# JARVIS-MoCap/JARVIS-HybridNet

Hardware: AMD Instinct MI355X
Metric: multi-view frames/s (12cam 1280x1024, 23kpt, 64^3 grid) (higher is better)
Workload: dtype f32; 1 GPU; BASELINE configs[2]: HybridNet 12-camera 1280x1024, 23 kpts, 64^3 grid, small/small; cameras=12, joints=23, grid=64, streams=3, parallelism=single GPU, 3 time batches in flight on 3 HIP streams, hipgraph=False

## Files before the change

### include/jarvis_hip.h

```cpp
#ifndef JARVIS_HIP_H
#define JARVIS_HIP_H
#include <stdint.h>

#ifdef __cplusplus
extern "C" {
#endif

#define JH_ABI_VERSION 4

const char* jh_last_error(void);
int jh_abi_version(void);

#define JH_PRECISION_DEFAULT (-1)
#define JH_PRECISION_F32 0
#define JH_PRECISION_BF16X3 1
#define JH_PRECISION_BF16X3_WIDE 2
int jh_set_precision(int mode);
int jh_get_precision(void);

typedef struct jh_params jh_params;
int jh_params_create(jh_params** out);
int jh_params_set(jh_params* p, const char* key, const float* host, int64_t numel);
void jh_params_destroy(jh_params* p);

typedef struct jh_efftrack jh_efftrack;
int jh_efftrack_create(const jh_params* p, const char* prefix, int model_size, int joints, int n,
                       int h, int w, int want_res1, jh_efftrack** out);
int jh_efftrack_forward(jh_efftrack* net, const float* x_dev, float* res1_dev, float* res2_dev,
                        void* stream);
int64_t jh_efftrack_launches(const jh_efftrack* net);
void jh_efftrack_destroy(jh_efftrack* net);

typedef struct jh_v2v jh_v2v;
int jh_v2v_create(const jh_params* p, const char* prefix, int joints, int t, int g, jh_v2v** out);
int jh_v2v_forward(jh_v2v* net, const float* x_dev, float* y_dev, void* stream);
void jh_v2v_destroy(jh_v2v* net);

int64_t jh_reproject_workspace_bytes(int cams, int joints, int hs, int grid_size);
int jh_reproject_forward(const float* heatmaps_padded_dev, int cams, int joints, int hs,
                         const int32_t* center3d_dev, const int32_t* center_hm_dev,
                         const float* cam_dev, const float* intr_dev, const float* dist_dev,
                         int grid_size, float grid_spacing, float* vol_dev, int32_t* idx_dev,
                         void* workspace_dev, int64_t workspace_bytes, void* stream);

int64_t jh_softargmax_workspace_bytes(int t, int joints, int gh);
int jh_softargmax(const float* v2v_out_dev, int t, int joints, int gh, float grid_spacing,
                  float roi_cube_size, const int32_t* center3d_dev, float* heatmap_final_dev,
                  float* points_dev, float* conf_dev, void* workspace_dev, int64_t workspace_bytes,
                  void* stream);

int jh_reproject_point(const float* points_dev, int npoints, int cams, const float* cam_dev,
                       const float* intr_dev, const float* dist_dev, float* uv_dev, void* stream);
int64_t jh_reconstruct_workspace_bytes(int cams);
int jh_reconstruct_point(const float* points2d_dev, const float* maxvals_dev, int cams,
                         const float* cam_dev, const float* intr_dev, const float* dist_dev,
                         float* point3d_dev, void* workspace_dev, int64_t workspace_bytes,
                         void* stream);

typedef struct jh_predictor jh_predictor;
typedef struct {
  int32_t num_cameras, num_joints;
  int32_t center_size;
  int32_t bbox;
  float roi_cube_size;
  float grid_spacing;
  int32_t center_model, kp_model;
  int32_t img_h, img_w;
  int32_t time_batch;
  int32_t time_batch_3d;
  int32_t cam_lo, cam_n;
  float mean[3], std[3];
  int32_t precision;
} jh_predictor_config;

int jh_predictor_create(const jh_params* center_params, const jh_params* hybrid_params,
                        const jh_predictor_config* cfg, jh_predictor** out);
void jh_predictor_destroy(jh_predictor* pr);
int64_t jh_predictor_launches(const jh_predictor* pr);
int64_t jh_predictor_device_bytes(const jh_predictor* pr);
int jh_predictor_precision(const jh_predictor* pr);

int jh_predictor_set_calibration(jh_predictor* pr, const float* cam_dev, const float* intr_dev,
                                 const float* dist_dev, void* stream);
int jh_predictor_set_calibration_frames(jh_predictor* pr, const float* cam_dev ,
                                        const float* intr_dev , const float* dist_dev ,
                                        void* stream);

int jh_predictor_set_centers(jh_predictor* pr, const float* centers_dev , void* stream);

int jh_predictor_stage_center(jh_predictor* pr, const float* frames_dev, float* det_dev,
                              void* stream);
int jh_predictor_stage_keypoints(jh_predictor* pr, const float* frames_dev,
                                 const float* det_all_dev, float* heat_dev, void* stream);
int jh_predictor_stage_3d(jh_predictor* pr, const float* heat_all_dev, int t0, float* points_dev,
                          float* conf_dev, int32_t* valid_dev, void* stream);
int jh_predictor_stage_keypoints_gathered(jh_predictor* pr, const void* frames_dev, int frames_u8,
                                          const float* det_gathered_dev, int n_blocks,
                                          float* heat_dev, void* stream);
int jh_predictor_stage_3d_blocks(jh_predictor* pr, const float* heat_blocks_dev, int n_blocks,
                                 int frames_per_block, int t_off, int t0, float* points_dev,
                                 float* conf_dev, int32_t* valid_dev, void* stream);
int jh_predictor_forward(jh_predictor* pr, const float* frames_dev, float* points_dev,
                         float* conf_dev, int32_t* valid_dev, void* stream);
int jh_predictor_set_graph_replay(jh_predictor* pr, int on);
int jh_predictor_graph_replay(const jh_predictor* pr);
int jh_predictor_stage_center_u8(jh_predictor* pr, const uint8_t* frames_dev, float* det_dev,
                                 void* stream);
int jh_predictor_stage_keypoints_u8(jh_predictor* pr, const uint8_t* frames_dev,
                                    const float* det_all_dev, float* heat_dev, void* stream);
int jh_predictor_forward_u8(jh_predictor* pr, const uint8_t* frames_dev, float* points_dev,
                            float* conf_dev, int32_t* valid_dev, void* stream);

#define JH_FRAME_RGB_F32 0
#define JH_FRAME_BGR_U8 1
#define JH_FRAME_I420 2
#define JH_FRAME_NV12 3
int jh_predictor_forward_yuv(jh_predictor* pr, const uint8_t* frames_dev, int format, float* points_dev,
                             float* conf_dev, int32_t* valid_dev, void* stream);

// ... 163 lines not shown
```

### jarvis-hybridnet_amd/_native.py

```python
import ctypes
import math
import os
from typing import NamedTuple

import torch

_HERE = os.path.dirname(os.path.abspath(__file__))
LIB_PATH = os.environ.get("JH_LIBRARY_PATH") or os.path.join(_HERE, "libjarvis_hip.so")
_lib = None

c_void_p, c_int, c_float, c_int64 = ctypes.c_void_p, ctypes.c_int, ctypes.c_float, ctypes.c_int64
c_char_p = ctypes.c_char_p


class PredictorConfig(ctypes.Structure):
    _fields_ = [("num_cameras", ctypes.c_int32), ("num_joints", ctypes.c_int32),
                ("center_size", ctypes.c_int32), ("bbox", ctypes.c_int32),
                ("roi_cube_size", c_float), ("grid_spacing", c_float),
                ("center_model", ctypes.c_int32), ("kp_model", ctypes.c_int32),
                ("img_h", ctypes.c_int32), ("img_w", ctypes.c_int32),
                ("time_batch", ctypes.c_int32), ("time_batch_3d", ctypes.c_int32),
                ("cam_lo", ctypes.c_int32),
                ("cam_n", ctypes.c_int32), ("mean", c_float * 3), ("std", c_float * 3),
                ("precision", ctypes.c_int32)]


class YuvSurfaceStruct(ctypes.Structure):
    _fields_ = [("image_stride", ctypes.c_int64), ("y_offset", ctypes.c_int64), ("y_pitch", ctypes.c_int64),
                ("u_offset", ctypes.c_int64), ("v_offset", ctypes.c_int64), ("c_pitch", ctypes.c_int64),
                ("c_step", ctypes.c_int32), ("matrix", ctypes.c_int32), ("range", ctypes.c_int32),
                ("reserved", ctypes.c_int32)]


assert ctypes.sizeof(YuvSurfaceStruct) == 64


class SensorSurfaceStruct(ctypes.Structure):
    _fields_ = [("image_stride", ctypes.c_int64), ("offset", ctypes.c_int64), ("pitch", ctypes.c_int64),
                ("pattern", ctypes.c_int32), ("reserved", ctypes.c_int32)]


assert ctypes.sizeof(SensorSurfaceStruct) == 32

class OpOperand(ctypes.Structure):
    _fields_ = [("in_sums_host", c_void_p), ("in_act", ctypes.c_int32), ("latency_class", ctypes.c_int32),
                ("want_stats", ctypes.c_int32), ("se_c", ctypes.c_int32), ("se_s", ctypes.c_int32),
                ("se_inv_hw", c_float), ("se_wr_host", c_void_p), ("se_br_host", c_void_p),
                ("se_we_host", c_void_p), ("se_be_host", c_void_p), ("se_pool_host", c_void_p)]


assert ctypes.sizeof(OpOperand) == 72

class SubjectsParamsStruct(ctypes.Structure):
    _fields_ = [("max_subjects", ctypes.c_int32), ("max_peaks", ctypes.c_int32), ("nms_radius", ctypes.c_int32),
                ("min_views", ctypes.c_int32), ("min_peak", c_float), ("max_error_px", c_float)]


assert ctypes.sizeof(SubjectsParamsStruct) == 24

ABI_VERSION = 4
assert ctypes.sizeof(PredictorConfig) == 84

_WORKSPACES = {}


def workspace(nbytes, device):
    key = (str(device), torch.cuda.current_stream(device).cuda_stream)
    bufs = _WORKSPACES.setdefault(key, [])
    if not bufs or bufs[-1].numel() < nbytes:
        bufs.append(torch.empty((max(int(nbytes), 256),), dtype=torch.uint8, device=device))
    return bufs[-1]


_SIGS = {
    "jh_last_error": (c_char_p, []),
    "jh_abi_version": (c_int, []),
    "jh_set_precision": (c_int, [c_int]),
    "jh_get_precision": (c_int, []),
    "jh_params_create": (c_int, [ctypes.POINTER(c_void_p)]),
    "jh_params_set": (c_int, [c_void_p, c_char_p, c_void_p, c_int64]),
    "jh_params_destroy": (None, [c_void_p]),
    "jh_efftrack_create": (c_int, [c_void_p, c_char_p, c_int, c_int, c_int, c_int, c_int, c_int,
                                   ctypes.POINTER(c_void_p)]),
    "jh_efftrack_forward": (c_int, [c_void_p, c_void_p, c_void_p, c_void_p, c_void_p]),
    "jh_efftrack_launches": (c_int64, [c_void_p]),
    "jh_efftrack_destroy": (None, [c_void_p]),
    "jh_v2v_create": (c_int, [c_void_p, c_char_p, c_int, c_int, c_int, ctypes.POINTER(c_void_p)]),
    "jh_v2v_forward": (c_int, [c_void_p, c_void_p, c_void_p, c_void_p]),
    "jh_v2v_destroy": (None, [c_void_p]),
    "jh_reproject_workspace_bytes": (c_int64, [c_int, c_int, c_int, c_int]),
    "jh_reproject_forward": (c_int, [c_void_p, c_int, c_int, c_int, c_void_p, c_void_p, c_void_p,
                                     c_void_p, c_void_p, c_int, c_float, c_void_p, c_void_p,
                                     c_void_p, c_int64, c_void_p]),
    "jh_softargmax_workspace_bytes": (c_int64, [c_int, c_int, c_int]),
    "jh_softargmax": (c_int, [c_void_p, c_int, c_int, c_int, c_float, c_float, c_void_p, c_void_p,
                              c_void_p, c_void_p, c_void_p, c_int64, c_void_p]),
    "jh_softargmax_spread_workspace_bytes": (c_int64, [c_int, c_int, c_int]),
    "jh_softargmax_spread": (c_int, [c_void_p, c_int, c_int, c_int, c_float, c_float, c_void_p, c_void_p,
                                     c_void_p, c_void_p, c_void_p, c_void_p, c_void_p, c_void_p, c_int64, c_void_p]),
    "jh_predictor_set_spread": (c_int, [c_void_p, c_int]),
    "jh_predictor_get_spread": (c_int, [c_void_p, c_void_p, c_void_p, c_void_p, c_void_p]),
    "jh_predictor_debug_v2v": (c_int, [c_void_p, c_void_p, c_void_p]),
    "jh_reproject_point": (c_int, [c_void_p, c_int, c_int, c_void_p, c_void_p, c_void_p, c_void_p,
                                   c_void_p]),
    "jh_reconstruct_workspace_bytes": (c_int64, [c_int]),
    "jh_reconstruct_point": (c_int, [c_void_p, c_void_p, c_int, c_void_p, c_void_p, c_void_p,
                                     c_void_p, c_void_p, c_int64, c_void_p]),
    "jh_predictor_create": (c_int, [c_void_p, c_void_p, ctypes.POINTER(PredictorConfig),
                                    ctypes.POINTER(c_void_p)]),
    "jh_predictor_destroy": (None, [c_void_p]),
    "jh_predictor_set_graph_replay": (c_int, [c_void_p, c_int]),
    "jh_predictor_graph_replay": (c_int, [c_void_p]),
    "jh_predictor_launches": (c_int64, [c_void_p]),
    "jh_predictor_device_bytes": (c_int64, [c_void_p]),
    "jh_predictor_precision": (c_int, [c_void_p]),
    "jh_predictor_set_calibration": (c_int, [c_void_p, c_void_p, c_void_p, c_void_p, c_void_p]),
    "jh_predictor_set_calibration_frames": (c_int, [c_void_p, c_void_p, c_void_p, c_void_p, c_void_p]),
    "jh_predictor_set_centers": (c_int, [c_void_p, c_void_p, c_void_p]),
    "jh_predictor_stage_center": (c_int, [c_void_p, c_void_p, c_void_p, c_void_p]),
    "jh_predictor_stage_keypoints": (c_int, [c_void_p, c_void_p, c_void_p, c_void_p, c_void_p]),
    "jh_predictor_stage_3d": (c_int, [c_void_p, c_void_p, c_int, c_void_p, c_void_p, c_void_p,
                                      c_void_p]),
    "jh_predictor_stage_keypoints_gathered": (c_int, [c_void_p, c_void_p, c_int, c_void_p, c_int, c_void_p,
                                                      c_void_p]),
    "jh_predictor_stage_3d_blocks": (c_int, [c_void_p, c_void_p, c_int, c_int, c_int, c_int, c_void_p,
                                             c_void_p, c_void_p, c_void_p]),
    "jh_profile_begin": (c_int, []),
    "jh_profile_end": (c_int, [ctypes.POINTER(c_int)]),
    "jh_profile_get": (c_int, [c_int, c_char_p, c_int, ctypes.POINTER(ctypes.c_double),
                               ctypes.POINTER(ctypes.c_double), ctypes.POINTER(ctypes.c_double)]),
    "jh_predictor_forward": (c_int, [c_void_p, c_void_p, c_void_p, c_void_p, c_void_p, c_void_p]),
    "jh_predictor_stage_center_u8": (c_int, [c_void_p, c_void_p, c_void_p, c_void_p]),
    "jh_predictor_stage_keypoints_u8": (c_int, [c_void_p, c_void_p, c_void_p, c_void_p, c_void_p]),
    "jh_predictor_forward_u8": (c_int, [c_void_p, c_void_p, c_void_p, c_void_p, c_void_p, c_void_p]),
    "jh_predictor_forward_yuv": (c_int, [c_void_p, c_void_p, c_int, c_void_p, c_void_p, c_void_p, c_void_p]),
    "jh_yuv_surface_check": (c_int, [ctypes.POINTER(YuvSurfaceStruct), c_int, c_int]),
    "jh_predictor_forward_surface": (c_int, [c_void_p, c_void_p, ctypes.POINTER(YuvSurfaceStruct), c_void_p, c_void_p,
                                             c_void_p, c_void_p, c_void_p]),
    "jh_predictor2d_forward_surface": (c_int, [c_void_p, c_void_p, ctypes.POINTER(YuvSurfaceStruct), c_void_p,
                                               c_void_p, c_void_p, c_void_p]),
    "jh_op_yuv_surface_to_bgr": (c_int, [c_void_p, ctypes.POINTER(YuvSurfaceStruct), c_int, c_int, c_int, c_void_p,
                                         c_void_p]),
    "jh_sensor_surface_check": (c_int, [ctypes.POINTER(SensorSurfaceStruct), c_int, c_int]),
    "jh_predictor_forward_sensor": (c_int, [c_void_p, c_void_p, ctypes.POINTER(SensorSurfaceStruct), c_void_p, c_void_p,
                                            c_void_p, c_void_p, c_void_p]),
    "jh_predictor2d_forward_sensor": (c_int, [c_void_p, c_void_p, ctypes.POINTER(SensorSurfaceStruct), c_void_p,
                                              c_void_p, c_void_p, c_void_p]),
    "jh_op_sensor_to_bgr": (c_int, [c_void_p, ctypes.POINTER(SensorSurfaceStruct), c_int, c_int, c_int, c_void_p,
                                    c_void_p]),
    "jh_predictor_forward_masked": (c_int, [c_void_p, c_void_p, c_int, c_void_p, c_void_p, c_void_p, c_void_p,
                                            c_void_p]),
    "jh_predictor_forward_images": (c_int, [c_void_p, ctypes.POINTER(c_void_p), c_int, c_int,
                                            ctypes.POINTER(YuvSurfaceStruct), ctypes.POINTER(SensorSurfaceStruct),
                                            c_void_p, c_void_p, c_void_p, c_void_p, c_void_p]),
    "jh_predictor2d_forward_images": (c_int, [c_void_p, ctypes.POINTER(c_void_p), c_int, c_int,
                                              ctypes.POINTER(YuvSurfaceStruct), ctypes.POINTER(SensorSurfaceStruct),
                                              c_void_p, c_void_p, c_void_p, c_void_p]),
    "jh_predictor_stage_keypoints_masked": (c_int, [c_void_p, c_void_p, c_int, c_void_p, c_void_p, c_void_p,
                                                    c_void_p]),
    "jh_predictor_stage_3d_masked": (c_int, [c_void_p, c_void_p, c_int, c_void_p, c_void_p, c_void_p, c_void_p,
                                             c_void_p]),
    "jh_predictor_debug_mask": (c_int, [c_void_p, c_void_p, c_void_p, c_void_p]),
    "jh_predictor_views2d": (c_int, [c_void_p, c_void_p, c_int] + [c_void_p] * 8),
    "jh_subjects_params_check": (c_int, [ctypes.POINTER(SubjectsParamsStruct)]),
    "jh_op_center_peaks": (c_int, [c_void_p, c_int, c_int, c_int, c_int, ctypes.POINTER(SubjectsParamsStruct), c_void_p,
                                   c_void_p, c_void_p]),
    "jh_op_associate_subjects": (c_int, [c_void_p, c_int, c_int, c_void_p, c_void_p, c_void_p, c_int, c_void_p,
                                         c_float, c_float, ctypes.POINTER(SubjectsParamsStruct), c_void_p, c_void_p,
                                         c_void_p, c_void_p, c_void_p]),
    "jh_predictor_detect_subjects": (c_int, [c_void_p, c_void_p, ctypes.POINTER(c_void_p), c_int, c_int,
                                             ctypes.POINTER(YuvSurfaceStruct), ctypes.POINTER(SensorSurfaceStruct),
                                             c_void_p, ctypes.POINTER(SubjectsParamsStruct), c_void_p, c_void_p,
# ... 372 lines not shown
```

### jarvis-hybridnet_amd/csrc/api.hip

```cpp
#include <cstring>
#include <memory>
#include "../../include/jarvis_hip.h"
#include <cstdlib>
#include "nets.h"
#include "bifpn_node.h"
#include "views2d.h"
#include "subjects.h"

namespace jh {
static thread_local std::string g_err;
void set_error(const std::string& msg) { g_err = msg; }
}

using namespace jh;

struct jh_params { ParamMap map; };
struct jh_efftrack { EffTrackPlan plan; };
struct jh_v2v { V2VPlan plan; };

namespace {

struct Scratch {
  std::vector<void*> ptrs;
  ~Scratch() { for (void* p : ptrs) (void)hipFree(p); }
// ... 93 lines not shown
  if (i < count) table[i] = c.p[i];
}
__global__ void copy_out_kernel(const float* __restrict__ gp, const float* __restrict__ gc,
                                const int* __restrict__ gv, float* __restrict__ points,
                                float* __restrict__ conf, int* __restrict__ valid, int n_pts, int n_conf,
                                int n_valid) {
  const int i = blockIdx.x * blockDim.x + threadIdx.x;
  if (i < n_pts) points[i] = gp[i];
  if (i < n_conf) conf[i] = gc[i];
  if (valid && i < n_valid) valid[i] = gv[i];
}

__global__ void pack_det_kernel(const float* __restrict__ pts2d, const float* __restrict__ maxvals,
                                float* __restrict__ det, int C) {
  const int c = threadIdx.x;
  if (c < C) {
    det[c * 3 + 0] = pts2d[c];
    det[c * 3 + 1] = pts2d[C + c];
    det[c * 3 + 2] = maxvals[c];
  }
}

}

extern "C" {

const char* jh_last_error(void) { return g_err.c_str(); }
int jh_abi_version(void) { return JH_ABI_VERSION; }

int jh_set_precision(int mode) {
  JH_REQUIRE(mode == JH_PRECISION_F32 || mode == JH_PRECISION_BF16X3 || mode == JH_PRECISION_BF16X3_WIDE,
             "unknown precision mode");
  set_precision_mode(mode);
  return 0;
}
int jh_get_precision(void) { return precision_mode(); }

int jh_params_create(jh_params** out) {
  *out = new jh_params();
  return 0;
}
int jh_params_set(jh_params* p, const char* key, const float* host, int64_t numel) {
  JH_REQUIRE(p && key && host && numel >= 0, "bad argument");
  p->map[key] = std::vector<float>(host, host + numel);
  return 0;
}
void jh_params_destroy(jh_params* p) { delete p; }

int jh_efftrack_create(const jh_params* p, const char* prefix, int model_size, int joints, int n,
                       int h, int w, int want_res1, jh_efftrack** out) {
  JH_REQUIRE(p && out, "bad argument");
  std::unique_ptr<jh_efftrack> net(new jh_efftrack());
  if (net->plan.build(p->map, prefix ? prefix : "", model_size, joints, n, h, w, want_res1 != 0)) return 1;
  *out = net.release();
  return 0;
}
int jh_efftrack_forward(jh_efftrack* net, const float* x_dev, float* res1_dev, float* res2_dev,
                        void* stream) {
  hipStream_t s = static_cast<hipStream_t>(stream);
  JH_REQUIRE(net && x_dev && res2_dev, "bad argument");
  JH_REQUIRE(!res1_dev || net->plan.res1.p, "res1 requested from a network created with want_res1 = 0");
  if (launch_to_channel_last(x_dev, net->plan.input, s)) return 1;
  if (net->plan.run(s)) return 1;
  if (res1_dev && launch_from_channel_last(net->plan.res1, res1_dev, s)) return 1;
  return launch_from_channel_last(net->plan.heat, res2_dev, s);
}
int64_t jh_efftrack_launches(const jh_efftrack* net) { return (int64_t)net->plan.launches(); }
void jh_efftrack_destroy(jh_efftrack* net) { delete net; }

int jh_v2v_create(const jh_params* p, const char* prefix, int joints, int t, int g, jh_v2v** out) {
  JH_REQUIRE(p && out, "bad argument");
  std::unique_ptr<jh_v2v> net(new jh_v2v());
  if (net->plan.build(p->map, prefix ? prefix : "", joints, t, g)) return 1;
  *out = net.release();
  return 0;
}
int jh_v2v_forward(jh_v2v* net, const float* x_dev, float* y_dev, void* stream) {
  hipStream_t s = static_cast<hipStream_t>(stream);
  if (launch_to_channel_last(x_dev, net->plan.input, s)) return 1;
  if (net->plan.run(s)) return 1;
  return launch_from_channel_last(net->plan.output, y_dev, s);
}
void jh_v2v_destroy(jh_v2v* net) { delete net; }

int64_t jh_reproject_workspace_bytes(int cams, int joints, int hs, int grid_size) {
  Carver c(nullptr, 0);
  ReproWs w;
  return (int64_t)carve_reproject(c, cams, joints, hs, grid_size, &w);
}

int jh_reproject_forward(const float* heatmaps_padded_dev, int cams, int joints, int hs,
                         const int32_t* center3d_dev, const int32_t* center_hm_dev,
                         const float* cam_dev, const float* intr_dev, const float* dist_dev,
                         int grid_size, float grid_spacing, float* vol_dev, int32_t* idx_dev,
                         void* workspace_dev, int64_t workspace_bytes, void* stream) {
  hipStream_t s = static_cast<hipStream_t>(stream);
  JH_REQUIRE(workspace_dev && workspace_bytes >= 0, "workspace (see jh_reproject_workspace_bytes)");
  JH_REQUIRE(grid_size > 0 && grid_size % 2 == 0, "grid size must be even");
  Carver c(workspace_dev, (size_t)workspace_bytes);
  ReproWs w;
  carve_reproject(c, cams, joints, hs, grid_size, &w);
  JH_REQUIRE(c.fits(), "workspace smaller than jh_reproject_workspace_bytes()");
  if (launch_to_channel_last(heatmaps_padded_dev, w.heat, s)) return 1;
  if (launch_reproject(Calib{cam_dev, intr_dev, dist_dev, 0}, center3d_dev, center_hm_dev, w.heat.p, w.coarse,
                       w.vol.p, idx_dev, 1, cams, grid_size, grid_spacing, hs, w.heat.Cp,
                       1, 0, nullptr, s)) return 1;
  return launch_from_channel_last(w.vol, vol_dev, s);
}

int64_t jh_softargmax_workspace_bytes(int t, int joints, int gh) {
  Carver c(nullptr, 0);
  SoftWs w;
  return (int64_t)carve_softargmax(c, t, joints, gh, &w);
}

int jh_softargmax(const float* v2v_out_dev, int t, int joints, int gh, float grid_spacing,
                  float roi_cube_size, const int32_t* center3d_dev, float* heatmap_final_dev,
                  float* points_dev, float* conf_dev, void* workspace_dev, int64_t workspace_bytes,
                  void* stream) {
  hipStream_t s = static_cast<hipStream_t>(stream);
  JH_REQUIRE(workspace_dev && workspace_bytes >= 0, "workspace (see jh_softargmax_workspace_bytes)");
  Carver c(workspace_dev, (size_t)workspace_bytes);
  SoftWs w;
  carve_softargmax(c, t, joints, gh, &w);
  JH_REQUIRE(c.fits(), "workspace smaller than jh_softargmax_workspace_bytes()");
  if (launch_to_channel_last(v2v_out_dev, w.x, s)) return 1;
  return launch_softargmax(w.x.p, center3d_dev, w.partial, w.pmax, points_dev, conf_dev,
                           heatmap_final_dev, t, joints, w.x.Cp, gh, grid_spacing, roi_cube_size, s);
}

int64_t jh_softargmax_spread_workspace_bytes(int t, int joints, int gh) {
  Carver c(nullptr, 0);
  SoftWs w;
  SoftargmaxSpread sp;
  carve_softargmax(c, t, joints, gh, &w);
  return (int64_t)carve_spread(c, t, w.x.Cp, &sp);
}

int jh_softargmax_spread(const float* v2v_out_dev, int t, int joints, int gh, float grid_spacing,
                         float roi_cube_size, const int32_t* center3d_dev, float* heatmap_final_dev,
                         float* points_dev, float* conf_dev, float* cov_dev, float* peak_dev, float* mass_dev,
                         void* workspace_dev, int64_t workspace_bytes, void* stream) {
  hipStream_t s = static_cast<hipStream_t>(stream);
  JH_REQUIRE(workspace_dev && workspace_bytes >= 0, "workspace (see jh_softargmax_spread_workspace_bytes)");
  JH_REQUIRE(cov_dev && peak_dev && mass_dev, "jh_softargmax_spread: null output pointer");
  Carver c(workspace_dev, (size_t)workspace_bytes);
  SoftWs w;
  SoftargmaxSpread sp;
  carve_softargmax(c, t, joints, gh, &w);
  carve_spread(c, t, w.x.Cp, &sp);
  JH_REQUIRE(c.fits(), "workspace smaller than jh_softargmax_spread_workspace_bytes()");
  sp.cov = cov_dev; sp.peak = peak_dev; sp.mass = mass_dev;
  if (launch_to_channel_last(v2v_out_dev, w.x, s)) return 1;
  return launch_softargmax(w.x.p, center3d_dev, w.partial, w.pmax, points_dev, conf_dev,
                           heatmap_final_dev, t, joints, w.x.Cp, gh, grid_spacing, roi_cube_size, s, &sp);
}

int jh_reproject_point(const float* points_dev, int npoints, int cams, const float* cam_dev,
                       const float* intr_dev, const float* dist_dev, float* uv_dev, void* stream) {
  return launch_project_points(points_dev, cam_dev, intr_dev, dist_dev, uv_dev, npoints, cams,
                               static_cast<hipStream_t>(stream));
}

int64_t jh_reconstruct_workspace_bytes(int cams) {
  Carver c(nullptr, 0);
  ReconWs w;
// ... 1408 lines not shown
```

### jarvis-hybridnet_amd/csrc/jh_common.h

```cpp
#pragma once
#include <hip/hip_runtime.h>
#include <cstdlib>
#include <cstdint>
#include <cstdio>
#include <cstring>
#include <string>
#include <vector>

namespace jh {

constexpr int kWave = 64;

#define JH_ENV_KNOB(name) ([]() -> int { static const int v = [] { const char* e = getenv(name); return e ? atoi(e) : -1; }(); return v; }())

inline int round_up(int v, int m) { return (v + m - 1) / m * m; }
inline int cpad(int c) { return round_up(c, 8); }

void set_error(const std::string& msg);
#define JH_CHECK_HIP(expr)                                                     \
  do {                                                                         \
    hipError_t _e = (expr);                                                    \
    if (_e != hipSuccess) {                                                    \
      jh::set_error(std::string(#expr) + ": " + hipGetErrorString(_e));        \
      return 1;                                                                \
// ... 181 lines not shown
__device__ __forceinline__ double exact_read(const double* src) { return (src[0] + src[1]) + src[2]; }
__device__ __forceinline__ void stat_add(double* st, float s1, float s2) {
  exact_add(st, (double)s1);
  exact_add(st + kLimbs, (double)s2);
}
__device__ __forceinline__ void exact_add_rounded(double* dst, double p) {
  const double a = fabs(p);
  double q;
  int slot;
  if (a < 0x1p5) { q = rint(p * 0x1p35) * 0x1p-35; slot = 2; }
  else if (a < 0x1p15) { q = rint(p * 0x1p25) * 0x1p-25; slot = 1; }
  else { q = rint(p * 0x1p15) * 0x1p-15; slot = 0; }
  if (q != 0.0) unsafeAtomicAdd(dst + slot, q);
}
__device__ __forceinline__ void stat_add(double* st, double s1, double s2) {
  exact_add_rounded(st, s1);
  exact_add_rounded(st + kLimbs, s2);
}
__device__ __forceinline__ void stat_acc(double& s1, double& s2, float v) {
  const double d = (double)v;
  s1 += d;
  s2 = fma(d, d, s2);
}
#endif

#if defined(__HIPCC__)
__device__ __forceinline__ unsigned xcd_linear(unsigned L, unsigned total) {
  const unsigned q = total >> 3, r = total & 7u, x = L & 7u, s = L >> 3;
  return x < r ? x * (q + 1) + s : r * (q + 1) + (x - r) * q + s;
}
__device__ __forceinline__ unsigned fd_div(unsigned x, const FastDiv& f) { return (__umulhi(x, f.mul) + x) >> f.shift; }
__device__ __forceinline__ BlockId xcd_block(const FastDiv& fgx, const FastDiv& fgy) {
  const unsigned gx = gridDim.x, gy = gridDim.y, gz = gridDim.z;
  const unsigned L = blockIdx.x + gx * (blockIdx.y + gy * blockIdx.z);
  const unsigned l = xcd_linear(L, gx * gy * gz);
  BlockId b;
  const unsigned l1 = fd_div(l, fgx);
  b.x = l - l1 * gx;
  b.z = fd_div(l1, fgy);
  b.y = l1 - b.z * gy;
  return b;
}
__device__ __forceinline__ BlockId xcd_block() {
  const unsigned gx = gridDim.x, gy = gridDim.y, gz = gridDim.z;
  const unsigned L = blockIdx.x + gx * (blockIdx.y + gy * blockIdx.z);
  unsigned l = xcd_linear(L, gx * gy * gz);
  BlockId b;
  b.x = l % gx; l /= gx;
  b.y = l % gy;
  b.z = l / gy;
  return b;
}
#endif

#if defined(__HIPCC__)
__device__ __forceinline__ float sum_xor16(float s) {
  const auto r = __builtin_amdgcn_permlane16_swap(__float_as_uint(s), __float_as_uint(s), false, false);
  return __uint_as_float(r[0]) + __uint_as_float(r[1]);
}
__device__ __forceinline__ float sum_xor32(float s) {
  const auto r = __builtin_amdgcn_permlane32_swap(__float_as_uint(s), __float_as_uint(s), false, false);
  return __uint_as_float(r[0]) + __uint_as_float(r[1]);
}
__device__ __forceinline__ double sum_xor16(double s) {
  const unsigned lo = (unsigned)__double2loint(s), hi = (unsigned)__double2hiint(s);
  const auto a = __builtin_amdgcn_permlane16_swap(lo, lo, false, false);
  const auto b = __builtin_amdgcn_permlane16_swap(hi, hi, false, false);
  return __hiloint2double((int)b[0], (int)a[0]) + __hiloint2double((int)b[1], (int)a[1]);
}
__device__ __forceinline__ double sum_xor32(double s) {
  const unsigned lo = (unsigned)__double2loint(s), hi = (unsigned)__double2hiint(s);
  const auto a = __builtin_amdgcn_permlane32_swap(lo, lo, false, false);
  const auto b = __builtin_amdgcn_permlane32_swap(hi, hi, false, false);
  return __hiloint2double((int)b[0], (int)a[0]) + __hiloint2double((int)b[1], (int)a[1]);
}
__device__ __forceinline__ float silu_fast(float v) { return v * __builtin_amdgcn_rcpf(1.f + __expf(-v)); }
#endif

struct NodeArgs;
int launch_bifpn_node(const NodeArgs& a, hipStream_t s);
int pack_wino_weights(int cin, int cout, const float* w, const float* b, ConvWeights* out);
int launch_conv3d_wino(const ConvWeights& w, const Act& x, const Act& y, double* stats, hipStream_t s,
                       const InNorm* in, int variant, const int* tables);
inline unsigned short bf16_rne(float f) {
  unsigned u;
  std::memcpy(&u, &f, 4);
  u += 0x7fffu + ((u >> 16) & 1u);
  return (unsigned short)(u >> 16);
}
inline float bf16_to_f32(unsigned short h) {
  const unsigned u = (unsigned)h << 16;
  float f;
  std::memcpy(&f, &u, 4);
  return f;
}
int pack_bf16x3_weights(int cin, int cout, const float* w, const float* b, ConvWeights* out);
int launch_conv3d_bf16x3(const ConvWeights& w, const Act& x, const Act& y, double* stats, hipStream_t s,
                         const InNorm* in);
int pack_deconv4_bf16x3_weights(int cin, int cout, const float* w, ConvWeights* out);
bool deconv4_bf16x3_eligible(int cout);
int launch_deconv4_bf16x3(const ConvWeights& w, const Act& x, const Act& y, hipStream_t s, const InNorm* in);
bool conv_bf16x3_eligible(const ConvDesc& d);
int pack_conv_bf16x3_weights(const ConvDesc& d, const float* w, const float* b, ConvWeights* out);
int launch_conv_bf16x3(const ConvDesc& d, const ConvWeights& w, const Act& x, const Act& y, double* stats,
                       hipStream_t s, const InNorm* in);
int precision_mode();
void set_precision_mode(int m);
void pack_stem_weights(const float* w_host, float* packed, int cout);
int launch_stem_conv(const Act& x, const float* w_dev, const Act& y, double* stats, hipStream_t s);
struct StemSource;
int launch_stem_conv_src(const StemSource& src, const Act& x, const float* w_dev, const Act& y, double* stats,
                         hipStream_t s);
int launch_deconv_c1(const Act& x, const double* stats, float inv_cnt, int in_act, const float* w,
                     const Act& y, hipStream_t s);

int launch_zero(void* p, size_t bytes, hipStream_t s);

int launch_to_channel_last(const float* src, const Act& dst, hipStream_t s);
int launch_from_channel_last(const Act& src, float* dst, hipStream_t s);

}
```

### jarvis-hybridnet_amd/csrc/nets.h

```cpp
#pragma once
#include <deque>
#include <functional>
#include <map>
#include <string>
#include <vector>
#include "jh_common.h"
#include "conv_layer.h"
#include "preprocess.h"

namespace jh {

int launch_reproject(const Calib& cal, const int* center3d, const int* center_hm, const float* heat, float2* coarse,
                     float* vol, int* idx_out, int T, int C, int G, float spacing, int hs, int Jp, int heat_pad,
                     int div255, const unsigned char* mask, hipStream_t s, const HeatLayout* layout = nullptr);
int launch_preprocess_resize(const void* frames, const FrameSource& src, float* out, int N, int H, int W, int S,
                             const float* mean, const float* stdv, hipStream_t s,
                             const void* const* frames_cell = nullptr);
int launch_preprocess_crop(const void* frames, const FrameSource& src, const int* center_hm, float* out, int T,
                           int Cloc, int C, int cam0, int H, int W, int B, const float* mean,
                           const float* stdv, hipStream_t s, const void* const* frames_cell = nullptr);
int launch_frames_to_bgr(const void* frames, const FrameSource& src, unsigned char* out, int N, int H, int W,
                         hipStream_t s);
int launch_center_argmax(const float* heat, float* det, int N, int Hh, int Wh, int Cp,
                         hipStream_t s);
// ... 21 lines not shown
                      int Gh, float spacing, float roi, hipStream_t s, const SoftargmaxSpread* spread = nullptr);

typedef std::map<std::string, std::vector<float>> ParamMap;

class Plan {
 public:
  ~Plan();
  int run(hipStream_t s);
  size_t launches() const { return ops_.size(); }
  size_t device_bytes() const { return bytes_; }
  int precision = precision_mode();
  int norm_block_kb = 0;

 protected:
  int alloc(void** p, size_t bytes);
  int new_act(int N, int D, int H, int W, int C, Act* out);
  size_t scratch(size_t doubles);
  int finish();
  double* sc(size_t off) const { return arena_ + off; }
  int upload(const std::vector<float>& host, float** dev);
  int get(const ParamMap& pm, const std::string& key, size_t numel, const float** out);

  struct Op { std::function<int(hipStream_t)> fn; std::string name; double flops, bytes; };
  std::vector<Op> ops_;
  void push(const std::string& name, double flops, double bytes, std::function<int(hipStream_t)> fn) {
    ops_.push_back(Op{std::move(fn), name, flops, bytes});
  }
  std::vector<void*> owned_;
  std::deque<ConvLayer> layers_;
  std::vector<ConvWeights> convs_;
  double* arena_ = nullptr;
  size_t arena_doubles_ = 0;
  size_t bytes_ = 0;

  int add_conv(const ParamMap& pm, const ConvDesc& d, const std::string& wkey,
               const std::string& bkey, bool transposed, const Act& x, const Act& y,
               const float* gate, bool want_stats, size_t* stats_off, long in_stats_off = -1,
               float in_inv = 0.f, int in_act = 0, const SeGate* se = nullptr, long se_pool_off = -1);
  void add_norm(const Act& x, size_t stats_off, int act, const float* r1, const float* r2,
                float* y, long pool_off, long r1_stats_off = -1);
};

struct Ref {
  Act a;
  long st = -1;
  float inv = 0.f;
  int act = 0;
};

class EffTrackPlan : public Plan {
 public:
  int build(const ParamMap& pm, const std::string& prefix, int size, int J, int N, int H, int W,
            bool want_res1 = false);
  bool stem_fusable = false;
  StemSource stem_src;
  void set_stem_traffic(double bytes);
  int stem_channels() const { return stem_ch_; }
  int node_rows = -1;
  Act input;
  Act heat;
  Act res1;
  int J = 0;
  int stem_op_ = -1, stem_ch_ = 16;

 private:
  int mbconv(const ParamMap& pm, const std::string& p, int stage, int k, int stride, int cin,
             int cout, int expand, Ref* x, Ref* out);
  void materialise(Ref* x);
  int lateral(const ParamMap& pm, const std::string& p, int cout, const Ref& x, Ref* out);
  int pool(const Ref& x, Ref* out);
  int node(const ParamMap& pm, const std::string& conv_prefix, int n_in, const Ref* ins,
           const int* modes, const float* w, int act, const Act& like, int cout, Ref* out,
           Ref* pooled = nullptr);
};

class V2VPlan : public Plan {
 public:
  int build(const ParamMap& pm, const std::string& prefix, int J, int T, int G);
  Act input;
  Act output;

 private:
  int res_block(const ParamMap& pm, const std::string& p, int c, const Act& x, const float* extra,
                Act* out, long x_stats = -1);
};

}
```

### jarvis-hybridnet_amd/csrc/nets.hip

```cpp
#include <cmath>
#include <cstring>
#include <cstdlib>
#include "nets.h"
#include "bifpn_node.h"

namespace jh {

Profiler& profiler() {
  static Profiler p;
  return p;
}
void Profiler::begin(const std::string& name, double flops, double bytes, hipStream_t s) {
  ProfRec r{name, flops, bytes, nullptr, nullptr, 0.f};
  (void)hipEventCreate(&r.e0);
  (void)hipEventCreate(&r.e1);
  (void)hipEventRecord(r.e0, s);
  recs.push_back(r);
}
void Profiler::end(hipStream_t s) { (void)hipEventRecord(recs.back().e1, s); }
int Profiler::finish() {
  JH_CHECK_HIP(hipDeviceSynchronize());
  for (auto& r : recs) {
    if (!r.e0) continue;
    JH_CHECK_HIP(hipEventElapsedTime(&r.ms, r.e0, r.e1));
// ... 390 lines not shown
      if (lateral(pm, p + "p5_down_channel", Wf, feats[2], &p5_in)) return 1;
      if (lateral(pm, p + "p4_down_channel_2", Wf, feats[1], &p4_in2)) return 1;
      if (lateral(pm, p + "p5_down_channel_2", Wf, feats[2], &p5_in2)) return 1;
    } else {
      p3_in = p3; p4_in = p4; p5_in = p5; p6_in = p6; p7_in = p7;
      p4_in2 = p4; p5_in2 = p5;
    }
    auto fnode = [&](const char* wname, int n_in, const Ref* ins, const int* modes, const Ref& like,
                     const char* conv, Ref* out, Ref* pooled = nullptr) -> int {
      const float* wp = nullptr;
      if (get(pm, p + wname, n_in, &wp)) return 1;
      float w[3];
      fuse_weights(wp, n_in, w);
      return node(pm, p + conv + ".", n_in, ins, modes, w, ACT_SILU, like.a, Wf, out, pooled);
    };
    const int m_up[2] = {FUSE_SAME, FUSE_UP2};
    const int m_dn3[3] = {FUSE_SAME, FUSE_SAME, FUSE_POOL2};
    const int m_dn2[2] = {FUSE_SAME, FUSE_POOL2};
    Ref p6_up, p5_up, p4_up, p3_out, p4_out, p5_out, p6_out, p7_out;
    { const Ref in[2] = {p6_in, p7_in}; if (fnode("p6_w1", 2, in, m_up, p6_in, "conv6_up", &p6_up)) return 1; }
    { const Ref in[2] = {p5_in, p6_up}; if (fnode("p5_w1", 2, in, m_up, p5_in, "conv5_up", &p5_up)) return 1; }
    { const Ref in[2] = {p4_in, p5_up}; if (fnode("p4_w1", 2, in, m_up, p4_in, "conv4_up", &p4_up)) return 1; }
    Ref p3_pool;
    { const Ref in[2] = {p3_in, p4_up}; if (fnode("p3_w1", 2, in, m_up, p3_in, "conv3_up", &p3_out, &p3_pool)) return 1; }
    const int m_same3[3] = {FUSE_SAME, FUSE_SAME, FUSE_SAME};
    Ref p4_pool;
    if (p3_pool.a.p) {
      const Ref in[3] = {p4_in2, p4_up, p3_pool};
      if (fnode("p4_w2", 3, in, m_same3, p4_in2, "conv4_down", &p4_out, &p4_pool)) return 1;
    } else {
      const Ref in[3] = {p4_in2, p4_up, p3_out};
      if (fnode("p4_w2", 3, in, m_dn3, p4_in2, "conv4_down", &p4_out)) return 1;
    }
    const bool more = cell + 1 < ss.cells;
    Ref p5_pool, p6_pool;
    if (p4_pool.a.p) {
      const Ref in[3] = {p5_in2, p5_up, p4_pool};
      if (fnode("p5_w2", 3, in, m_same3, p5_in2, "conv5_down", &p5_out, more ? &p5_pool : nullptr)) return 1;
    } else {
      const Ref in[3] = {p5_in2, p5_up, p4_out};
      if (fnode("p5_w2", 3, in, m_dn3, p5_in2, "conv5_down", &p5_out)) return 1;
    }
    if (more) {
      if (p5_pool.a.p) {
        const Ref in[3] = {p6_in, p6_up, p5_pool};
        if (fnode("p6_w2", 3, in, m_same3, p6_in, "conv6_down", &p6_out, &p6_pool)) return 1;
      } else {
        const Ref in[3] = {p6_in, p6_up, p5_out};
        if (fnode("p6_w2", 3, in, m_dn3, p6_in, "conv6_down", &p6_out)) return 1;
      }
      if (p6_pool.a.p) {
        const int m_same2[2] = {FUSE_SAME, FUSE_SAME};
        const Ref in[2] = {p7_in, p6_pool};
        if (fnode("p7_w2", 2, in, m_same2, p7_in, "conv7_down", &p7_out)) return 1;
      } else {
        const Ref in[2] = {p7_in, p6_out};
        if (fnode("p7_w2", 2, in, m_dn2, p7_in, "conv7_down", &p7_out)) return 1;
      }
    }
    p3 = p3_out; p4 = p4_out; p5 = p5_out; p6 = p6_out; p7 = p7_out;
  }

  const float* wc = nullptr;
  if (get(pm, pre + "weights_cat", 3, &wc)) return 1;
  float w[3], sum = 0.f;
  for (int i = 0; i < 3; ++i) { w[i] = wc[i] > 20.f ? wc[i] : log1pf(expf(wc[i])); sum += w[i]; }
  for (int i = 0; i < 3; ++i) w[i] = w[i] / (sum + 0.0001f);
  const Ref hin[3] = {p3, p4, p5};
  const int hmodes[3] = {FUSE_SAME, FUSE_UP2, FUSE_UP4};
  Ref mid;
  if (node(pm, pre + "first_conv.", 3, hin, hmodes, w, ACT_NONE, p3.a, ss.head, &mid)) return 1;
  if (new_act(N, 1, mid.a.H * 2, mid.a.W * 2, J, &heat)) return 1;
  if (want_res1) {
    if (new_act(N, 1, mid.a.H, mid.a.W, J, &res1)) return 1;
    if (add_conv(pm, conv_desc(2, 3, 1, 1, ss.head, J), pre + "final_conv1.weight", "", false, mid.a,
                 res1, nullptr, false, nullptr, mid.st, mid.inv, ACT_NONE)) return 1;
  }
  if (add_conv(pm, deconv2d_k4s2p1_desc(ss.head, J), pre + "deconv1.weight", "", true, mid.a, heat,
               nullptr, false, nullptr, mid.st, mid.inv, ACT_NONE)) return 1;
  return finish();
}

int V2VPlan::res_block(const ParamMap& pm, const std::string& p, int c, const Act& x,
                       const float* extra, Act* out, long x_stats) {
  Act a;
  if (new_act(x.N, x.D, x.H, x.W, c, &a)) return 1;
  size_t s1 = 0, s2 = 0;
  const float inv = 1.f / (float)(x.D * x.H * x.W);
  if (add_conv(pm, conv_desc(3, 3, 1, 1, c, c), p + "res_branch.0.weight", p + "res_branch.0.bias",
               false, x, a, nullptr, true, &s1, x_stats, inv, ACT_RELU)) return 1;
  if (new_act(x.N, x.D, x.H, x.W, c, out)) return 1;
  if (add_conv(pm, conv_desc(3, 3, 1, 1, c, c), p + "res_branch.3.weight", p + "res_branch.3.bias",
               false, a, *out, nullptr, true, &s2, (long)s1, 1.f / (float)(x.D * x.H * x.W),
               ACT_RELU)) return 1;
  add_norm(*out, s2, ACT_RELU, x.p, extra, out->p, -1, x_stats);
  return 0;
}

int V2VPlan::build(const ParamMap& pm, const std::string& pre, int J, int T, int G) {
  JH_REQUIRE(G % 4 == 0, "grid size must be a multiple of 4");
  const int Gh = G / 2, Gq = G / 4;
  if (new_act(T, G, G, G, J, &input)) return 1;
  Act f0, f1, skip, e0, e1, u0, d1;
  size_t st = 0;
  if (new_act(T, Gh, Gh, Gh, 2 * J, &f0)) return 1;
  if (add_conv(pm, conv_desc(3, 3, 2, 1, J, 2 * J), pre + "front_layers.0.block.0.weight",
               pre + "front_layers.0.block.0.bias", false, input, f0, nullptr, true, &st)) return 1;
  if (res_block(pm, pre + "front_layers.1.", 2 * J, f0, nullptr, &f1, (long)st)) return 1;
  const std::string e = pre + "encoder_decoder.";
  if (res_block(pm, e + "skip_res1.", 2 * J, f1, nullptr, &skip)) return 1;
  if (new_act(T, Gq, Gq, Gq, 4 * J, &e0)) return 1;
  if (add_conv(pm, conv_desc(3, 2, 2, 0, 2 * J, 4 * J), e + "encoder_pool1.block.0.weight",
               e + "encoder_pool1.block.0.bias", false, f1, e0, nullptr, true, &st)) return 1;
  if (res_block(pm, e + "mid_res.", 4 * J, e0, nullptr, &e1, (long)st)) return 1;
  if (new_act(T, Gh, Gh, Gh, 2 * J, &u0)) return 1;
  if (add_conv(pm, deconv3d_k2s2_desc(4 * J, 2 * J), e + "decoder_upsample1.block.0.weight",
               e + "decoder_upsample1.block.0.bias", true, e1, u0, nullptr, true, &st)) return 1;
  if (res_block(pm, e + "decoder_res1.", 2 * J, u0, skip.p, &d1, (long)st)) return 1;
  if (new_act(T, Gh, Gh, Gh, J, &output)) return 1;
  if (add_conv(pm, conv_desc(3, 1, 1, 0, 2 * J, J), pre + "output_layer.weight",
               pre + "output_layer.bias", false, d1, output, nullptr, false, nullptr)) return 1;
  return finish();
}

}
```

Baseline: 2161 multi-view frames/s.

## Fold V2V residual-block norms into the final 1x1x1 output conv kernel

Skips the instance-norm/ReLU/residual-add passes of the skip_res1 and decoder_res1 blocks. A new MFMA kernel recomputes those normalised activations on the fly from raw conv outputs and stats, then applies the 1x1x1 output conv. This removes two full elementwise read/write passes over half-resolution volumes and their launches. In exchange the fused kernel reads four input tensors, and the path is enabled by default for J<=32 and G%8==0.

```diff
diff --git a/include/jarvis_hip.h b/include/jarvis_hip.h
--- a/include/jarvis_hip.h
+++ b/include/jarvis_hip.h
@@ -35,6 +35,7 @@
 int jh_v2v_create(const jh_params* p, const char* prefix, int joints, int t, int g, jh_v2v** out);
 int jh_v2v_forward(jh_v2v* net, const float* x_dev, float* y_dev, void* stream);
 void jh_v2v_destroy(jh_v2v* net);
+int jh_v2v_fold(int joints, int t, int g, int* folded);
 
 int64_t jh_reproject_workspace_bytes(int cams, int joints, int hs, int grid_size);
 int jh_reproject_forward(const float* heatmaps_padded_dev, int cams, int joints, int hs,
diff --git a/jarvis-hybridnet_amd/_native.py b/jarvis-hybridnet_amd/_native.py
--- a/jarvis-hybridnet_amd/_native.py
+++ b/jarvis-hybridnet_amd/_native.py
@@ -88,6 +88,7 @@
     "jh_v2v_create": (c_int, [c_void_p, c_char_p, c_int, c_int, c_int, ctypes.POINTER(c_void_p)]),
     "jh_v2v_forward": (c_int, [c_void_p, c_void_p, c_void_p, c_void_p]),
     "jh_v2v_destroy": (None, [c_void_p]),
+    "jh_v2v_fold": (c_int, [c_int, c_int, c_int, ctypes.POINTER(c_int)]),
     "jh_reproject_workspace_bytes": (c_int64, [c_int, c_int, c_int, c_int]),
     "jh_reproject_forward": (c_int, [c_void_p, c_int, c_int, c_int, c_void_p, c_void_p, c_void_p,
                                      c_void_p, c_void_p, c_int, c_float, c_void_p, c_void_p,
diff --git a/jarvis-hybridnet_amd/csrc/api.hip b/jarvis-hybridnet_amd/csrc/api.hip
--- a/jarvis-hybridnet_amd/csrc/api.hip
+++ b/jarvis-hybridnet_amd/csrc/api.hip
@@ -199,6 +199,11 @@
   return launch_from_channel_last(net->plan.output, y_dev, s);
 }
 void jh_v2v_destroy(jh_v2v* net) { delete net; }
+int jh_v2v_fold(int joints, int t, int g, int* folded) {
+  JH_REQUIRE(joints >= 1 && t >= 1 && g >= 4 && g % 4 == 0 && folded, "jh_v2v_fold: bad argument");
+  *folded = v2v_fold_applies(joints, g) ? 1 : 0;
+  return 0;
+}
 
 int64_t jh_reproject_workspace_bytes(int cams, int joints, int hs, int grid_size) {
   Carver c(nullptr, 0);
diff --git a/jarvis-hybridnet_amd/csrc/conv3d_out_fold.hip b/jarvis-hybridnet_amd/csrc/conv3d_out_fold.hip
--- /dev/null
+++ b/jarvis-hybridnet_amd/csrc/conv3d_out_fold.hip
@@ -0,0 +1,208 @@
+#include "conv_mfma.h"
+
+namespace jh {
+
+namespace {
+typedef float of4 __attribute__((ext_vector_type(4)));
+typedef unsigned ou4 __attribute__((ext_vector_type(4)));
+
+struct OutFoldArgs {
+  const float *r_dec, *u0, *r_skip, *f1;
+  const double *st_dec, *st_u0, *st_skip;
+  const float *w, *bias;
+  float* y;
+  double eps;
+  int P, Cp, cout_p, cout_p16;
+};
+
+template <int K8, int NCB, bool PF>
+__global__ __launch_bounds__(256, 2) void conv3d_out_fold_kernel(const OutFoldArgs a, int rb_per_wave) {
+  constexpr int KW = (K8 + 1) / 2;
+  __shared__ __attribute__((aligned(16))) float nrm_s[3][2][64];
+  const int tid = threadIdx.x;
+  const int lane = tid & 63;
+  const int wave = __builtin_amdgcn_readfirstlane(tid >> 6);
+  const int px = lane & 15, kq = lane >> 4;
+  const int n = blockIdx.y;
+  const int P = a.P, Cp = a.Cp;
+
+  if (tid < 3 * Cp) {
+    const int slot = tid / Cp, c = tid - slot * Cp;
+    const double* base = slot == 0 ? a.st_dec : (slot == 1 ? a.st_u0 : a.st_skip);
+    const double* st = base + ((size_t)n * Cp + c) * kStatW;
+    const double mu = exact_read(st) / (double)P;
+    double var = exact_read(st + kLimbs) / (double)P - mu * mu;
+    if (var < 0.0) var = 0.0;
+    nrm_s[slot][0][c] = (float)mu;
+    nrm_s[slot][1][c] = (float)(1.0 / sqrt(var + a.eps));
+  }
+  __syncthreads();
+  const int nrb = P >> 4;
+  const int rb0 = (blockIdx.x * 4 + wave) * rb_per_wave;
+  const int rb1 = min(nrb, rb0 + rb_per_wave);
+  if (rb0 >= nrb) return;
+
+  of4 mu[3][KW], rs[3][KW];
+#pragma unroll
+  for (int u = 0; u < KW; ++u) {
+    const bool in = 16 * u + 4 * kq < Cp;
+#pragma unroll
+    for (int sl = 0; sl < 3; ++sl) {
+      mu[sl][u] = in ? *reinterpret_cast<const of4*>(&nrm_s[sl][0][16 * u + 4 * kq]) : (of4){0.f, 0.f, 0.f, 0.f};
+      rs[sl][u] = in ? *reinterpret_cast<const of4*>(&nrm_s[sl][1][16 * u + 4 * kq]) : (of4){1.f, 1.f, 1.f, 1.f};
+    }
+  }
+
+  float2 bw[K8][NCB];
+#pragma unroll
+  for (int k8 = 0; k8 < K8; ++k8)
+#pragma unroll
+    for (int cb = 0; cb < NCB; ++cb)
+      bw[k8][cb] = *reinterpret_cast<const float2*>(a.w + ((size_t)(k8 * NCB + cb) * 64 + lane) * 2);
+
+  const size_t img = (size_t)n * P * Cp;
+  const int img_bytes = (int)((size_t)P * Cp * 4);
+  const __amdgpu_buffer_rsrc_t rs_dec = __builtin_amdgcn_make_buffer_rsrc(const_cast<float*>(a.r_dec + img), 0, img_bytes, 0x00020000);
+  const __amdgpu_buffer_rsrc_t rs_u0 = __builtin_amdgcn_make_buffer_rsrc(const_cast<float*>(a.u0 + img), 0, img_bytes, 0x00020000);
+  const __amdgpu_buffer_rsrc_t rs_skip = __builtin_amdgcn_make_buffer_rsrc(const_cast<float*>(a.r_skip + img), 0, img_bytes, 0x00020000);
+  const __amdgpu_buffer_rsrc_t rs_f1 = __builtin_amdgcn_make_buffer_rsrc(const_cast<float*>(a.f1 + img), 0, img_bytes, 0x00020000);
+  int xoff[KW];
+#pragma unroll
+  for (int u = 0; u < KW; ++u)
+    xoff[u] = 16 * u + 4 * kq < Cp ? (px * Cp + 16 * u + 4 * kq) * 4 : (int)0x80000000;
+  const int xrb = 16 * Cp * 4;
+  const int j = lane & 3;
+  const __amdgpu_buffer_rsrc_t yrs = __builtin_amdgcn_make_buffer_rsrc(
+      a.y + (size_t)n * P * a.cout_p, 0, (int)((size_t)P * a.cout_p * 4), 0x00020000);
+  int yoff[NCB];
+  float bv[NCB];
+#pragma unroll
+  for (int cb = 0; cb < NCB; ++cb) {
+    const int c0 = 16 * cb + (px & ~3), ch = 16 * cb + px;
+    yoff[cb] = c0 < a.cout_p ? ((kq * 4 + j) * a.cout_p + c0) * 4 : (int)0x80000000;
+    bv[cb] = (a.bias && ch < a.cout_p16) ? a.bias[ch] : 0.f;
+  }
+  const int yrb = 16 * a.cout_p * 4;
+
+  struct Row { of4 d[KW], u[KW], s[KW], f[KW]; };
+  auto load = [&](int rb, Row& r) __attribute__((always_inline)) {
+#pragma unroll
+    for (int u = 0; u < KW; ++u) {
+      r.d[u] = __builtin_bit_cast(of4, __builtin_amdgcn_raw_buffer_load_b128(rs_dec, xoff[u], rb * xrb, 0));
+      r.u[u] = __builtin_bit_cast(of4, __builtin_amdgcn_raw_buffer_load_b128(rs_u0, xoff[u], rb * xrb, 0));
+      r.s[u] = __builtin_bit_cast(of4, __builtin_amdgcn_raw_buffer_load_b128(rs_skip, xoff[u], rb * xrb, 0));
+      r.f[u] = __builtin_bit_cast(of4, __builtin_amdgcn_raw_buffer_load_b128(rs_f1, xoff[u], rb * xrb, 0));
+    }
+  };
+  auto compute = [&](int rb, const Row& r) __attribute__((always_inline)) {
+    float2 av[2 * KW];
+#pragma unroll
+    for (int u = 0; u < KW; ++u) {
+      of4 t = (r.d[u] - mu[0][u]) * rs[0][u];
+      of4 e = (r.u[u] - mu[1][u]) * rs[1][u];
+      of4 s = (r.s[u] - mu[2][u]) * rs[2][u];
+#pragma unroll
+      for (int i = 0; i < 4; ++i) e[i] = fmaxf(e[i], 0.f);
+      t += e;
+      s += r.f[u];
+#pragma unroll
+      for (int i = 0; i < 4; ++i) { t[i] = fmaxf(t[i], 0.f); s[i] = fmaxf(s[i], 0.f); }
+      const of4 d1 = t + s;
+      const auto x0 = __builtin_amdgcn_permlane16_swap(__float_as_uint(d1[0]), __float_as_uint(d1[2]), false, false);
+      const auto x1 = __builtin_amdgcn_permlane16_swap(__float_as_uint(d1[1]), __float_as_uint(d1[3]), false, false);
+      const auto z0 = __builtin_amdgcn_permlane32_swap(x0[0], x0[1], false, false);
+      const auto z1 = __builtin_amdgcn_permlane32_swap(x1[0], x1[1], false, false);
+      av[2 * u] = make_float2(__uint_as_float(z0[0]), __uint_as_float(z1[0]));
+      av[2 * u + 1] = make_float2(__uint_as_float(z0[1]), __uint_as_float(z1[1]));
+    }
+    f32x4 acc[NCB];
+#pragma unroll
+    for (int cb = 0; cb < NCB; ++cb) acc[cb] = (f32x4){0.f, 0.f, 0.f, 0.f};
+#pragma unroll
+    for (int k8 = 0; k8 < K8; ++k8) {
+#pragma unroll
+      for (int cb = 0; cb < NCB; ++cb)
+        acc[cb] = __builtin_amdgcn_mfma_f32_16x16x4f32(av[k8].x, bw[k8][cb].x, acc[cb], 0, 0, 0);
+#pragma unroll
+      for (int cb = 0; cb < NCB; ++cb)
+        acc[cb] = __builtin_amdgcn_mfma_f32_16x16x4f32(av[k8].y, bw[k8][cb].y, acc[cb], 0, 0, 0);
+    }
+#pragma unroll
+    for (int cb = 0; cb < NCB; ++cb) {
+      float v[4];
+#pragma unroll
+      for (int i = 0; i < 4; ++i) v[i] = acc[cb][i] + bv[cb];
+      {
+        float x, y;
+        x = (j & 1) ? v[0] : v[1]; y = quad_xor1(x); if (j & 1) v[0] = y; else v[1] = y;
+        x = (j & 1) ? v[2] : v[3]; y = quad_xor1(x); if (j & 1) v[2] = y; else v[3] = y;
+        x = (j & 2) ? v[0] : v[2]; y = quad_xor2(x); if (j & 2) v[0] = y; else v[2] = y;
+        x = (j & 2) ? v[1] : v[3]; y = quad_xor2(x); if (j & 2) v[1] = y; else v[3] = y;
+      }
+      const of4 o = (of4){v[0], v[1], v[2], v[3]};
+      __builtin_amdgcn_raw_buffer_store_b128(__builtin_bit_cast(ou4, o), yrs, yoff[cb], rb * yrb, 0);
+    }
+  };
+
+  if constexpr (PF) {
+    Row ra, rb_;
+    int rb = rb0;
+    load(rb, ra);
+    while (true) {
+      if (rb + 1 < rb1) load(rb + 1, rb_);
+      compute(rb, ra);
+      if (++rb >= rb1) break;
+      if (rb + 1 < rb1) load(rb + 1, ra);
+      compute(rb, rb_);
+      if (++rb >= rb1) break;
+    }
+  } else {
+    for (int rb = rb0; rb < rb1; ++rb) {
+      Row r;
+      load(rb, r);
+      compute(rb, r);
+    }
+  }
+}
+}
+
+bool v2v_fold_shape(int J, int G) {
+  return J >= 1 && J <= 32 && G >= 8 && G % 8 == 0;
+}
+
+bool v2v_fold_applies(int J, int G) {
+  const char* e = getenv("JH_V2V_FOLD");
+  return (e ? atoi(e) : 1) != 0 && v2v_fold_shape(J, G);
+}
+
+int launch_conv3d_out_fold(const ConvWeights& w, const Act& r_dec, const double* st_dec, const float* u0,
+                           const double* st_u0, const float* r_skip, const double* st_skip, const float* f1,
+                           const Act& y, hipStream_t s) {
+  const size_t P = r_dec.pixels();
+  JH_REQUIRE(w.layout == WeightLayout::Plain && w.cin_p == r_dec.Cp && w.cout_p16 == round_up(y.C, 16) && w.bias,
+             "output fold: the packed weights of the 1 x 1 x 1 layer");
+  JH_REQUIRE(r_dec.Cp <= 64 && w.cout_p16 <= 32 && (r_dec.Cp > 32) == (w.cout_p16 > 16) && P % 16 == 0 &&
+             P * r_dec.Cp * 4 < ((size_t)1 << 31), "output fold: shape (v2v_fold_shape)");
+  JH_REQUIRE(y.N == r_dec.N && y.pixels() == P && y.Cp == cpad(y.C) && st_dec && st_u0 && st_skip && u0 && r_skip && f1,
+             "output fold: operands");
+  OutFoldArgs a;
+  a.r_dec = r_dec.p; a.u0 = u0; a.r_skip = r_skip; a.f1 = f1;
+  a.st_dec = st_dec; a.st_u0 = st_u0; a.st_skip = st_skip;
+  a.w = w.w; a.bias = w.bias; a.y = y.p; a.eps = 1e-5;
+  a.P = (int)P; a.Cp = r_dec.Cp; a.cout_p = y.Cp; a.cout_p16 = w.cout_p16;
+  const int nrb = (int)(P / 16);
+  const int rbw = (int)std::max<long>(1, std::min<long>(16, (long)nrb * r_dec.N / 4096));
+  const dim3 grid((nrb + 4 * rbw - 1) / (4 * rbw), r_dec.N);
+  const int k8 = a.Cp / 8;
+#define JH_OF(K8V, NCBV)                                                                                       \
+  if (k8 == K8V) {                                                                                             \
+    hipLaunchKernelGGL((conv3d_out_fold_kernel<K8V, NCBV, (K8V == 6)>), grid, dim3(256), 0, s, a, rbw);        \
+    JH_CHECK_HIP(hipGetLastError());                                                                           \
+    return 0;                                                                                                  \
+  }
+  JH_OF(1, 1) JH_OF(2, 1) JH_OF(3, 1) JH_OF(4, 1) JH_OF(5, 2) JH_OF(6, 2) JH_OF(7, 2) JH_OF(8, 2)
+#undef JH_OF
+  JH_REQUIRE(false, "output fold: no kernel for this channel count");
+}
+
+}
diff --git a/jarvis-hybridnet_amd/csrc/jh_common.h b/jarvis-hybridnet_amd/csrc/jh_common.h
--- a/jarvis-hybridnet_amd/csrc/jh_common.h
+++ b/jarvis-hybridnet_amd/csrc/jh_common.h
@@ -287,6 +287,11 @@
 int pack_wino_weights(int cin, int cout, const float* w, const float* b, ConvWeights* out);
 int launch_conv3d_wino(const ConvWeights& w, const Act& x, const Act& y, double* stats, hipStream_t s,
                        const InNorm* in, int variant, const int* tables);
+bool v2v_fold_shape(int J, int G);
+bool v2v_fold_applies(int J, int G);
+int launch_conv3d_out_fold(const ConvWeights& w, const Act& r_dec, const double* st_dec, const float* u0,
+                           const double* st_u0, const float* r_skip, const double* st_skip, const float* f1,
+                           const Act& y, hipStream_t s);
 inline unsigned short bf16_rne(float f) {
   unsigned u;
   std::memcpy(&u, &f, 4);
diff --git a/jarvis-hybridnet_amd/csrc/nets.h b/jarvis-hybridnet_amd/csrc/nets.h
--- a/jarvis-hybridnet_amd/csrc/nets.h
+++ b/jarvis-hybridnet_amd/csrc/nets.h
@@ -127,7 +127,7 @@
 
  private:
   int res_block(const ParamMap& pm, const std::string& p, int c, const Act& x, const float* extra,
-                Act* out, long x_stats = -1);
+                Act* out, long x_stats = -1, size_t* raw_stats = nullptr);
 };
 
 }
diff --git a/jarvis-hybridnet_amd/csrc/nets.hip b/jarvis-hybridnet_amd/csrc/nets.hip
--- a/jarvis-hybridnet_amd/csrc/nets.hip
+++ b/jarvis-hybridnet_amd/csrc/nets.hip
@@ -496,7 +496,7 @@
 }
 
 int V2VPlan::res_block(const ParamMap& pm, const std::string& p, int c, const Act& x,
-                       const float* extra, Act* out, long x_stats) {
+                       const float* extra, Act* out, long x_stats, size_t* raw_stats) {
   Act a;
   if (new_act(x.N, x.D, x.H, x.W, c, &a)) return 1;
   size_t s1 = 0, s2 = 0;
@@ -507,6 +507,7 @@
   if (add_conv(pm, conv_desc(3, 3, 1, 1, c, c), p + "res_branch.3.weight", p + "res_branch.3.bias",
                false, a, *out, nullptr, true, &s2, (long)s1, 1.f / (float)(x.D * x.H * x.W),
                ACT_RELU)) return 1;
+  if (raw_stats) { *raw_stats = s2; return 0; }
   add_norm(*out, s2, ACT_RELU, x.p, extra, out->p, -1, x_stats);
   return 0;
 }
@@ -522,7 +523,9 @@
                pre + "front_layers.0.block.0.bias", false, input, f0, nullptr, true, &st)) return 1;
   if (res_block(pm, pre + "front_layers.1.", 2 * J, f0, nullptr, &f1, (long)st)) return 1;
   const std::string e = pre + "encoder_decoder.";
-  if (res_block(pm, e + "skip_res1.", 2 * J, f1, nullptr, &skip)) return 1;
+  const bool fold = v2v_fold_applies(J, G);
+  size_t st_skip = 0, st_dec = 0;
+  if (res_block(pm, e + "skip_res1.", 2 * J, f1, nullptr, &skip, -1, fold ? &st_skip : nullptr)) return 1;
   if (new_act(T, Gq, Gq, Gq, 4 * J, &e0)) return 1;
   if (add_conv(pm, conv_desc(3, 2, 2, 0, 2 * J, 4 * J), e + "encoder_pool1.block.0.weight",
                e + "encoder_pool1.block.0.bias", false, f1, e0, nullptr, true, &st)) return 1;
@@ -530,10 +533,33 @@
   if (new_act(T, Gh, Gh, Gh, 2 * J, &u0)) return 1;
   if (add_conv(pm, deconv3d_k2s2_desc(4 * J, 2 * J), e + "decoder_upsample1.block.0.weight",
                e + "decoder_upsample1.block.0.bias", true, e1, u0, nullptr, true, &st)) return 1;
-  if (res_block(pm, e + "decoder_res1.", 2 * J, u0, skip.p, &d1, (long)st)) return 1;
+  const size_t st_u0 = st;
+  if (res_block(pm, e + "decoder_res1.", 2 * J, u0, skip.p, &d1, (long)st, fold ? &st_dec : nullptr)) return 1;
   if (new_act(T, Gh, Gh, Gh, J, &output)) return 1;
-  if (add_conv(pm, conv_desc(3, 1, 1, 0, 2 * J, J), pre + "output_layer.weight",
-               pre + "output_layer.bias", false, d1, output, nullptr, false, nullptr)) return 1;
+  if (!fold) {
+    if (add_conv(pm, conv_desc(3, 1, 1, 0, 2 * J, J), pre + "output_layer.weight",
+                 pre + "output_layer.bias", false, d1, output, nullptr, false, nullptr)) return 1;
+    return finish();
+  }
+  const float *w = nullptr, *b = nullptr;
+  if (get(pm, pre + "output_layer.weight", (size_t)2 * J * J, &w)) return 1;
+  if (get(pm, pre + "output_layer.bias", J, &b)) return 1;
+  ConvUse use;
+  use.desc = conv_desc(3, 1, 1, 0, 2 * J, J);
+  use.has_bias = true; use.precision = precision; use.in_px = d1.Cp;
+  layers_.emplace_back();
+  const ConvLayer* layer = &layers_.back();
+  if (make_conv_layer(use, w, b, Gh, Gh, Gh, &layers_.back())) return 1;
+  JH_REQUIRE(layer->choice.form == ConvForm::Mfma && layer->choice.layout == WeightLayout::Plain,
+             "output fold: the 1 x 1 x 1 layer's weight layout");
+  bytes_ += layer->device_bytes();
+  const double vox = (double)T * d1.pixels();
+  char nm[96];
+  snprintf(nm, sizeof nm, "conv3d_k1s1fold_%dx%d@%d", 2 * J, J, Gh);
+  push(nm, 2.0 * vox * 2 * J * J, 4.0 * (vox * (4.0 * d1.Cp + output.Cp) + 2.0 * J * J),
+       [this, layer, d1, u0, skip, f1, st_dec, st_u0, st_skip](hipStream_t s) {
+    return launch_conv3d_out_fold(layer->w, d1, sc(st_dec), u0.p, sc(st_u0), skip.p, sc(st_skip), f1.p, output, s);
+  });
   return finish();
 }
 
```

New measurement: 2189 multi-view frames/s, median of 6. +1.3%, better.
